# Septimus4/semi-supervised-image-processing

Hardware: AMD Instinct MI355X
Metric: images/sec semi-supervised train step, 224x224 bs=256, 1/2/4/8 MI355X (higher is better)
Workload: dtype bf16; 1 GPU; semi_consistency_resnet18_224; model=resnet18, global_batch=256, per_gpu_batch=256, labeled_per_gpu=128, unlabeled_per_gpu=128, image_size=224, parallelism=dp1

## Files before the change

semi-supervised-image-processing_amd/csrc/optim.hip:

```cpp
#include "ssip_common.h"

namespace {

struct AdamC {
  float decay, w1, b2, eps, step_size, bc2_sqrt, grad_scale;
};

__device__ __forceinline__ void adamw_math(float& pi, float& mi, float& vi, float graw, const AdamC& c) {
#pragma clang fp contract(off)
  const float gi = graw * c.grad_scale;
  pi = pi * c.decay;
  mi = (c.w1 < 0.5f) ? mi + c.w1 * (gi - mi) : gi - (gi - mi) * (1.f - c.w1);
  vi = vi * c.b2 + (1.f - c.b2) * gi * gi;
  const float denom = sqrtf(vi) / c.bc2_sqrt + c.eps;
  pi = pi - c.step_size * (mi / denom);
}

__device__ __forceinline__ void adamw_scalar(long i, float* __restrict__ p, const float* __restrict__ g,
                                             float* __restrict__ m, float* __restrict__ v, const AdamC& c) {
  float pi = p[i], mi = m[i], vi = v[i];
  adamw_math(pi, mi, vi, g[i], c);
  p[i] = pi;
  m[i] = mi;
  v[i] = vi;
}

__device__ __forceinline__ void adamw_range(long n, float* __restrict__ p, const float* __restrict__ g,
                                            float* __restrict__ m, float* __restrict__ v, const AdamC& c) {
  const long tid = blockIdx.x * (long)blockDim.x + threadIdx.x, nt = (long)gridDim.x * blockDim.x;
  const uintptr_t a = reinterpret_cast<uintptr_t>(p) & 15;
  const bool vec = (reinterpret_cast<uintptr_t>(g) & 15) == a && (reinterpret_cast<uintptr_t>(m) & 15) == a &&
                   (reinterpret_cast<uintptr_t>(v) & 15) == a && (a & 3) == 0;
  const long head = vec ? min(n, (long)(((16 - a) & 15) >> 2)) : n;
  for (long i = tid; i < head; i += nt) adamw_scalar(i, p, g, m, v, c);
  if (!vec) return;
  const long nv = (n - head) >> 2;
  float4* __restrict__ p4 = reinterpret_cast<float4*>(p + head);
  const float4* __restrict__ g4 = reinterpret_cast<const float4*>(g + head);
  float4* __restrict__ m4 = reinterpret_cast<float4*>(m + head);
  float4* __restrict__ v4 = reinterpret_cast<float4*>(v + head);
  for (long j = tid; j < nv; j += 2 * nt) {
    const long j1 = j + nt < nv ? j + nt : j;
    float4 pp[2] = {p4[j], p4[j1]}, mm[2] = {m4[j], m4[j1]}, vv[2] = {v4[j], v4[j1]};
    const float4 gg[2] = {g4[j], g4[j1]};
    asm volatile("" ::: "memory");
#pragma unroll
    for (int u = 0; u < 2; ++u) {
      adamw_math(pp[u].x, mm[u].x, vv[u].x, gg[u].x, c);
      adamw_math(pp[u].y, mm[u].y, vv[u].y, gg[u].y, c);
      adamw_math(pp[u].z, mm[u].z, vv[u].z, gg[u].z, c);
      adamw_math(pp[u].w, mm[u].w, vv[u].w, gg[u].w, c);
    }
    p4[j] = pp[0];
    m4[j] = mm[0];
    v4[j] = vv[0];
    if (j1 != j) {
      p4[j1] = pp[1];
      m4[j1] = mm[1];
      v4[j1] = vv[1];
    }
  }
  for (long i = head + (nv << 2) + tid; i < n; i += nt) adamw_scalar(i, p, g, m, v, c);
}

__global__ void adamw_kernel(long n, float* __restrict__ p, const float* __restrict__ g, float* __restrict__ m,
                             float* __restrict__ v, float lr, float b1, float b2, float eps, float wd, float step_size,
                             float bc2_sqrt, float grad_scale) {
  const AdamC c{1.f - lr * wd, 1.f - b1, b2, eps, step_size, bc2_sqrt, grad_scale};
  adamw_range(n, p, g, m, v, c);
}

__global__ void adamw_sched_kernel(double* sched, double b1, double b2) {
  const double t = sched[1] + 1.0;
  sched[1] = t;
  sched[2] = sched[0] / (1.0 - pow(b1, t));
  sched[3] = sqrt(1.0 - pow(b2, t));
  sched[5] = 1.0 - pow(b1, t + 1.0);
  sched[6] = sqrt(1.0 - pow(b2, t + 1.0));
}

__global__ void adamw_dev_kernel(long n, float* __restrict__ p, const float* __restrict__ g, float* __restrict__ m,
                                 float* __restrict__ v, double* sched, float b1, float b2, float eps, float wd,
                                 float grad_scale, int advance) {
  double t = sched[1], ss = sched[2], bc = sched[3];
  if (advance) {
    t += 1.0;
    const double c1 = sched[5];
    if (c1 != 0.0) {
      ss = sched[0] / c1;
      bc = sched[6];
    } else {
      ss = sched[0] / (1.0 - pow((double)b1, t));
      bc = sqrt(1.0 - pow((double)b2, t));
    }
  }
  const float lr = (float)sched[0];
  const AdamC c{1.f - lr * wd, 1.f - b1, b2, eps, (float)ss, (float)bc, grad_scale};
  adamw_range(n, p, g, m, v, c);
  if (advance) {
    __syncthreads();
    if (threadIdx.x != 0) return;
    unsigned long long* cnt = reinterpret_cast<unsigned long long*>(sched + 4);
    const unsigned long long old = __hip_atomic_fetch_add(cnt, 1ull, __ATOMIC_RELAXED, __HIP_MEMORY_SCOPE_AGENT);
    if (old == gridDim.x - 1) {
      sched[1] = t;
      sched[2] = ss;
      sched[3] = bc;
      sched[5] = 1.0 - pow((double)b1, t + 1.0);
      sched[6] = sqrt(1.0 - pow((double)b2, t + 1.0));
      __hip_atomic_store(cnt, 0ull, __ATOMIC_RELAXED, __HIP_MEMORY_SCOPE_AGENT);
    }
  }
}

template <typename T>
__global__ void weight_prep_kernel(int K, int C, int R, int S, int Cp, int Sp, const float* __restrict__ w,
                                   T* __restrict__ krsc, T* __restrict__ crsk) {
  const long total = (long)K * R * Sp * Cp;
  for (long i = blockIdx.x * (long)blockDim.x + threadIdx.x; i < total; i += (long)gridDim.x * blockDim.x) {
    const int c = (int)(i % Cp);
    long t = i / Cp;
    const int s = (int)(t % Sp);
    t /= Sp;
    const int r = (int)(t % R);
    const int k = (int)(t / R);
    const float v = (c < C && s < S) ? w[(((long)k * C + c) * R + r) * S + s] : 0.f;
    const T tv = from_f32<T>(v);
    if (krsc) krsc[i] = tv;
    if (crsk) crsk[(((long)c * R + r) * Sp + s) * K + k] = tv;
  }
}

struct WprepTable {
  ssip_wprep it[SSIP_WPREP_MAX];
  int tile_start[SSIP_WPREP_MAX + 1];
  int count;
  int xcd;
};

template <typename T>
__global__ void __launch_bounds__(256) weight_prep_batch_kernel(const WprepTable tab) {
  __shared__ float tile[64][65];
  int b = blockIdx.x, idx = 0;
  if (tab.xcd) {
    const int nb = gridDim.x, xcd = b & 7, q = nb >> 3, r = nb & 7;
    b = xcd * q + min(xcd, r) + (b >> 3);
  }
  while (idx + 1 < tab.count && b >= tab.tile_start[idx + 1]) ++idx;
  const ssip_wprep& e = tab.it[idx];
  b -= tab.tile_start[idx];
  const int rs = b % (e.R * e.Sp);
  b /= e.R * e.Sp;
  const int r = rs / e.Sp, s = rs - r * e.Sp;
  const int ctiles = (e.Cp + 63) / 64;
  const int k0 = (b / ctiles) * 64, c0 = (b % ctiles) * 64;
  const int tx = threadIdx.x & 63, ty = threadIdx.x >> 6;
  T* krsc = static_cast<T*>(e.w_krsc);
  T* crsk = static_cast<T*>(e.w_crsk);
  float vals[16];
#pragma unroll
  for (int q = 0; q < 16; ++q) {
    const int k = k0 + ty + 4 * q, c = c0 + tx;
    vals[q] = (k < e.K && c < e.C && s < e.S) ? e.w_kcrs[(((long)k * e.C + c) * e.R + r) * e.S + s] : 0.f;
  }
#pragma unroll
  for (int q = 0; q < 16; ++q) {
    const int k = k0 + ty + 4 * q;
    float v = vals[q];
    if (e.kscale && k < e.K && c0 + tx < e.C && s < e.S) v *= e.kscale[k];
    tile[ty + 4 * q][tx] = v;
  }
  __syncthreads();
  if (krsc) {
    for (int kk = ty; kk < 64; kk += 4) {
      const int k = k0 + kk, c = c0 + tx;
      if (k < e.K && c < e.Cp) krsc[(((long)k * e.R + r) * e.Sp + s) * e.Cp + c] = from_f32<T>(tile[kk][tx]);
    }
  }
  if (crsk) {
    for (int cc = ty; cc < 64; cc += 4) {
      const int c = c0 + cc, k = k0 + tx;
      if (k < e.K && c < e.Cp) crsk[(((long)c * e.R + r) * e.Sp + s) * e.K + k] = from_f32<T>(tile[tx][cc]);
    }
  }
}

}

extern "C" {

int ssip_adamw(int64_t n, float* param, const float* grad, float* exp_avg, float* exp_avg_sq, float lr, float beta1,
               float beta2, float eps, float weight_decay, int64_t step, float grad_scale, void* stream) {
  SSIP_REQUIRE(n > 0 && param && grad && exp_avg && exp_avg_sq && step >= 1, SSIP_ERR_ARG, "ssip_adamw: bad arguments");
  const double bc1 = 1.0 - pow((double)beta1, (double)step);
  const double bc2 = 1.0 - pow((double)beta2, (double)step);
  const float step_size = (float)((double)lr / bc1);
  const float bc2_sqrt = (float)sqrt(bc2);
  long blocks = (n + 1023) / 1024;
  if (blocks > 8192) blocks = 8192;
  SSIP_KLAUNCH(adamw_kernel, dim3((int)blocks), dim3(256), 0, (hipStream_t)stream, (long)n, param, grad, exp_avg,
                     exp_avg_sq, lr, beta1, beta2, eps, weight_decay, step_size, bc2_sqrt, grad_scale);
  return ::ssip::check_launch("adamw");
}

int ssip_adamw_sched_step(double* sched, float beta1, float beta2, void* stream) {
  SSIP_REQUIRE(sched, SSIP_ERR_ARG, "ssip_adamw_sched_step: null schedule");
  SSIP_KLAUNCH(adamw_sched_kernel, dim3(1), dim3(1), 0, (hipStream_t)stream, sched, (double)beta1,
                     (double)beta2);
  return ::ssip::check_launch("adamw_sched");
}

int ssip_adamw_dev(int64_t n, float* param, const float* grad, float* exp_avg, float* exp_avg_sq, double* sched,
                   float beta1, float beta2, float eps, float weight_decay, float grad_scale, int advance,
                   void* stream) {
  SSIP_REQUIRE(n > 0 && param && grad && exp_avg && exp_avg_sq && sched, SSIP_ERR_ARG,
               "ssip_adamw_dev: bad arguments");
  long blocks = (n + 1023) / 1024;
  if (blocks > 2048) blocks = 2048;
  SSIP_KLAUNCH(adamw_dev_kernel, dim3((int)blocks), dim3(256), 0, (hipStream_t)stream, (long)n, param, grad,
                     exp_avg, exp_avg_sq, sched, beta1, beta2, eps, weight_decay, grad_scale, advance ? 1 : 0);
  return ::ssip::check_launch("adamw_dev");
}

int ssip_weight_prep(int dtype, int K, int C, int R, int S, int Cp, int Sp, const float* w_kcrs, void* w_krsc,
                     void* w_crsk, void* stream) {
  SSIP_REQUIRE(K > 0 && C > 0 && R > 0 && S > 0 && Cp >= C && Sp >= S && w_kcrs && (w_krsc || w_crsk), SSIP_ERR_ARG,
               "ssip_weight_prep: bad arguments");
  const long total = (long)K * R * Sp * Cp;
  long blocks = (total + 255) / 256;
  if (blocks > 8192) blocks = 8192;
  SSIP_DISPATCH_DTYPE(dtype, T, {
    SSIP_KLAUNCH(weight_prep_kernel<T>, dim3((int)blocks), dim3(256), 0, (hipStream_t)stream, K, C, R, S, Cp, Sp,
                       w_kcrs, (T*)w_krsc, (T*)w_crsk);
  });
  return ::ssip::check_launch("weight_prep");
}

}

extern "C" int ssip_weight_prep_batch(int dtype, int count, const ssip_wprep* items, void* stream) {
  SSIP_REQUIRE(count >= 0 && count <= SSIP_WPREP_MAX && (count == 0 || items), SSIP_ERR_ARG,
               "ssip_weight_prep_batch: count must be 0..%d", SSIP_WPREP_MAX);
  if (count == 0) return SSIP_OK;
  WprepTable tab;
  memset(&tab, 0, sizeof(tab));
  tab.count = count;
  int tiles = 0;
  for (int i = 0; i < count; ++i) {
    const ssip_wprep& e = items[i];
    SSIP_REQUIRE(e.K > 0 && e.C > 0 && e.R > 0 && e.S > 0 && e.Cp >= e.C && e.Sp >= e.S && e.w_kcrs &&
                     (e.w_krsc || e.w_crsk),
                 SSIP_ERR_ARG, "ssip_weight_prep_batch: bad item %d", i);
    tab.it[i] = e;
    tab.tile_start[i] = tiles;
    tiles += ((e.K + 63) / 64) * ((e.Cp + 63) / 64) * e.R * e.Sp;
  }
  tab.tile_start[count] = tiles;
  tab.xcd = 1;
  SSIP_DISPATCH_DTYPE(dtype, T, {
    SSIP_KLAUNCH(weight_prep_batch_kernel<T>, dim3(tiles), dim3(256), 0, (hipStream_t)stream, tab);
  });
  return ::ssip::check_launch("weight_prep_batch");
}

namespace {
struct CounterTable {
  int64_t* p[SSIP_COUNTERS_MAX];
};

__global__ void counters_add_kernel(CounterTable t, int count, int64_t delta) {
  const int i = threadIdx.x;
  if (i < count) t.p[i][0] += delta;
}
}

extern "C" int ssip_counters_add(int count, int64_t* const* ptrs, int64_t delta, void* stream) {
  SSIP_REQUIRE(count >= 0 && count <= SSIP_COUNTERS_MAX && (count == 0 || ptrs), SSIP_ERR_ARG,
               "ssip_counters_add: count must be 0..%d", SSIP_COUNTERS_MAX);
  if (count == 0) return SSIP_OK;
  CounterTable t;
  for (int i = 0; i < count; ++i) {
    SSIP_REQUIRE(ptrs[i], SSIP_ERR_ARG, "ssip_counters_add: null counter %d", i);
    t.p[i] = ptrs[i];
  }
  SSIP_KLAUNCH(counters_add_kernel, dim3(1), dim3(64), 0, (hipStream_t)stream, t, count, delta);
  return ::ssip::check_launch("counters_add");
}
```

Before: 44180 images/s.

## Retile batched weight prep to read contiguous KCRS rows with float4 and vectorized stores

The batched weight-layout kernel now tiles over K and C only, with every R,S position inside one tile. Each block loads whole contiguous KCRS rows with aligned float4 reads into a padded LDS tile. It then writes the KRSC and CRSK layouts with 16-byte packed stores where alignment allows. This replaces strided scalar gathers (one tile per r,s position) with coalesced vector traffic and fewer, larger blocks, at the cost of more complex index walking and LDS-size-driven tile selection on the host.

```diff
diff --git a/semi-supervised-image-processing_amd/csrc/optim.hip b/semi-supervised-image-processing_amd/csrc/optim.hip
--- a/semi-supervised-image-processing_amd/csrc/optim.hip
+++ b/semi-supervised-image-processing_amd/csrc/optim.hip
@@ -131,57 +131,167 @@
   }
 }
 
+constexpr int kWprepLdsElems = 9472;
+constexpr int kWprepMaxVec = 10;
+
 struct WprepTable {
   ssip_wprep it[SSIP_WPREP_MAX];
   int tile_start[SSIP_WPREP_MAX + 1];
+  unsigned char tk[SSIP_WPREP_MAX], tc[SSIP_WPREP_MAX];
   int count;
-  int xcd;
 };
+
+__host__ __device__ inline int wprep_kstride(int c, int rs, int esize) {
+  int ks = c * rs;
+  while (esize == 2 ? (ks & 3) != 2 : !(ks & 1)) ++ks;
+  return ks;
+}
+
+__host__ __device__ inline bool wprep_tile_fits(int tk, int tc, int C, int rs, int esize) {
+  const int c = tc < C ? tc : C;
+  return tk * wprep_kstride(c, rs, esize) <= kWprepLdsElems && tk * ((c * rs + 6) / 4) <= 256 * kWprepMaxVec;
+}
+
+template <typename T, int W>
+struct alignas(sizeof(T) * W) WprepPack {
+  T e[W];
+};
+
+struct WprepWalk {
+  int hi, r, s, lo, dhi, dr, ds, dlo, R, Sp, n;
+  __device__ __forceinline__ WprepWalk(int v, int R_, int Sp_, int n_) : R(R_), Sp(Sp_), n(n_) {
+    split(v, hi, r, s, lo);
+    split(256, dhi, dr, ds, dlo);
+  }
+  __device__ __forceinline__ void split(int v, int& h, int& r_, int& s_, int& l) const {
+    l = v % n;
+    v /= n;
+    s_ = v % Sp;
+    v /= Sp;
+    r_ = v % R;
+    h = v / R;
+  }
+  __device__ __forceinline__ void next() {
+    lo += dlo;
+    if (lo >= n) lo -= n, ++s;
+    s += ds;
+    if (s >= Sp) s -= Sp, ++r;
+    r += dr;
+    if (r >= R) r -= R, ++hi;
+    hi += dhi;
+  }
+};
+
+template <typename T, int W>
+__device__ __forceinline__ void wprep_store_krsc(const ssip_wprep& e, const T* tile, int ks, int k0, int c0, int tke,
+                                                 int nc, int wc) {
+  T* krsc = static_cast<T*>(e.w_krsc);
+  const int RS = e.R * e.S, cv = wc / W, nv = tke * e.R * e.Sp * cv;
+  WprepWalk w(threadIdx.x, e.R, e.Sp, cv);
+  for (int v = threadIdx.x; v < nv; v += 256, w.next()) {
+    const int cl = w.lo * W;
+    const T* src = tile + w.hi * ks + w.r * e.S + w.s;
+    WprepPack<T, W> p;
+#pragma unroll
+    for (int j = 0; j < W; ++j) p.e[j] = (w.s < e.S && cl + j < nc) ? src[(cl + j) * RS] : from_f32<T>(0.f);
+    *reinterpret_cast<WprepPack<T, W>*>(krsc + (((k0 + w.hi) * e.R + w.r) * e.Sp + w.s) * e.Cp + c0 + cl) = p;
+  }
+}
+
+template <typename T, int W>
+__device__ __forceinline__ void wprep_store_crsk(const ssip_wprep& e, const T* tile, int ks, int k0, int c0, int tke,
+                                                 int nc, int wc) {
+  T* crsk = static_cast<T*>(e.w_crsk);
+  const int RS = e.R * e.S, kv = tke / W, nv = wc * e.R * e.Sp * kv;
+  WprepWalk w(threadIdx.x, e.R, e.Sp, kv);
+  for (int v = threadIdx.x; v < nv; v += 256, w.next()) {
+    const int kk = w.lo * W;
+    const T* src = tile + kk * ks + w.hi * RS + w.r * e.S + w.s;
+    const bool in = w.s < e.S && w.hi < nc;
+    WprepPack<T, W> p;
+#pragma unroll
+    for (int j = 0; j < W; ++j) p.e[j] = in ? src[j * ks] : from_f32<T>(0.f);
+    *reinterpret_cast<WprepPack<T, W>*>(crsk + (((c0 + w.hi) * e.R + w.r) * e.Sp + w.s) * e.K + k0 + kk) = p;
+  }
+}
 
 template <typename T>
 __global__ void __launch_bounds__(256) weight_prep_batch_kernel(const WprepTable tab) {
-  __shared__ float tile[64][65];
+  __shared__ T tile[kWprepLdsElems];
+  constexpr int VE = 16 / (int)sizeof(T);
   int b = blockIdx.x, idx = 0;
-  if (tab.xcd) {
+  {
     const int nb = gridDim.x, xcd = b & 7, q = nb >> 3, r = nb & 7;
     b = xcd * q + min(xcd, r) + (b >> 3);
   }
   while (idx + 1 < tab.count && b >= tab.tile_start[idx + 1]) ++idx;
   const ssip_wprep& e = tab.it[idx];
   b -= tab.tile_start[idx];
-  const int rs = b % (e.R * e.Sp);
-  b /= e.R * e.Sp;
-  const int r = rs / e.Sp, s = rs - r * e.Sp;
-  const int ctiles = (e.Cp + 63) / 64;
-  const int k0 = (b / ctiles) * 64, c0 = (b % ctiles) * 64;
-  const int tx = threadIdx.x & 63, ty = threadIdx.x >> 6;
-  T* krsc = static_cast<T*>(e.w_krsc);
-  T* crsk = static_cast<T*>(e.w_crsk);
-  float vals[16];
-#pragma unroll
-  for (int q = 0; q < 16; ++q) {
-    const int k = k0 + ty + 4 * q, c = c0 + tx;
-    vals[q] = (k < e.K && c < e.C && s < e.S) ? e.w_kcrs[(((long)k * e.C + c) * e.R + r) * e.S + s] : 0.f;
-  }
-#pragma unroll
-  for (int q = 0; q < 16; ++q) {
-    const int k = k0 + ty + 4 * q;
-    float v = vals[q];
-    if (e.kscale && k < e.K && c0 + tx < e.C && s < e.S) v *= e.kscale[k];
-    tile[ty + 4 * q][tx] = v;
+  const int TK = tab.tk[idx], TC = tab.tc[idx];
+  const int ktiles = (e.K + TK - 1) / TK;
+  const int k0 = (b % ktiles) * TK, c0 = (b / ktiles) * TC;
+  const int RS = e.R * e.S;
+  const int tke = min(TK, e.K - k0);
+  const int nc = max(0, min(TC, e.C - c0));
+  const int wc = min(TC, e.Cp - c0);
+  const int rl = nc * RS;
+  const int ks = wprep_kstride(min(TC, e.C), RS, (int)sizeof(T));
+  const int spr = (rl + 6) >> 2, nslots = tke * spr;
+  const int total = e.K * e.C * RS;
+  const int mis = (int)((reinterpret_cast<uintptr_t>(e.w_kcrs) >> 2) & 3);
+  float4 vals[kWprepMaxVec];
+  float sc[kWprepMaxVec];
+  const int kk0 = threadIdx.x / spr, j0 = threadIdx.x - kk0 * spr, dk = 256 / spr, dj = 256 - dk * spr;
+  int kk = kk0, j = j0;
+#pragma unroll
+  for (int q = 0; q < kWprepMaxVec; ++q) {
+    vals[q] = make_float4(0.f, 0.f, 0.f, 0.f);
+    sc[q] = 1.f;
+    const int lo = ((k0 + kk) * e.C + c0) * RS;
+    const int e0 = lo - ((lo + mis) & 3) + 4 * j;
+    if (threadIdx.x + 256 * q < nslots && e0 < lo + rl) {
+      if (e.kscale) sc[q] = e.kscale[k0 + kk];
+      if (e0 >= 0 && e0 + 4 <= total) {
+        vals[q] = *reinterpret_cast<const float4*>(e.w_kcrs + e0);
+      } else {
+        if (e0 >= 0 && e0 < total) vals[q].x = e.w_kcrs[e0];
+        if (e0 + 1 >= 0 && e0 + 1 < total) vals[q].y = e.w_kcrs[e0 + 1];
+        if (e0 + 2 >= 0 && e0 + 2 < total) vals[q].z = e.w_kcrs[e0 + 2];
+        if (e0 + 3 >= 0 && e0 + 3 < total) vals[q].w = e.w_kcrs[e0 + 3];
+      }
+    }
+    j += dj;
+    if (j >= spr) j -= spr, ++kk;
+    kk += dk;
+  }
+  kk = kk0, j = j0;
+#pragma unroll
+  for (int q = 0; q < kWprepMaxVec; ++q) {
+    if (threadIdx.x + 256 * q < nslots) {
+      const int lo = ((k0 + kk) * e.C + c0) * RS;
+      const int off = 4 * j - ((lo + mis) & 3);
+      const float v4[4] = {vals[q].x, vals[q].y, vals[q].z, vals[q].w};
+#pragma unroll
+      for (int i = 0; i < 4; ++i) {
+        if (off + i >= 0 && off + i < rl) tile[kk * ks + off + i] = from_f32<T>(e.kscale ? v4[i] * sc[q] : v4[i]);
+      }
+    }
+    j += dj;
+    if (j >= spr) j -= spr, ++kk;
+    kk += dk;
   }
   __syncthreads();
-  if (krsc) {
-    for (int kk = ty; kk < 64; kk += 4) {
-      const int k = k0 + kk, c = c0 + tx;
-      if (k < e.K && c < e.Cp) krsc[(((long)k * e.R + r) * e.Sp + s) * e.Cp + c] = from_f32<T>(tile[kk][tx]);
-    }
-  }
-  if (crsk) {
-    for (int cc = ty; cc < 64; cc += 4) {
-      const int c = c0 + cc, k = k0 + tx;
-      if (k < e.K && c < e.Cp) crsk[(((long)c * e.R + r) * e.Sp + s) * e.K + k] = from_f32<T>(tile[tx][cc]);
-    }
+  if (e.w_krsc) {
+    if (wc % VE == 0 && e.Cp % VE == 0 && (reinterpret_cast<uintptr_t>(e.w_krsc) & 15) == 0)
+      wprep_store_krsc<T, VE>(e, tile, ks, k0, c0, tke, nc, wc);
+    else
+      wprep_store_krsc<T, 1>(e, tile, ks, k0, c0, tke, nc, wc);
+  }
+  if (e.w_crsk) {
+    if (TK % VE == 0 && e.K % VE == 0 && (reinterpret_cast<uintptr_t>(e.w_crsk) & 15) == 0)
+      wprep_store_crsk<T, VE>(e, tile, ks, k0, c0, tke, nc, wc);
+    else
+      wprep_store_crsk<T, 1>(e, tile, ks, k0, c0, tke, nc, wc);
   }
 }
 
@@ -242,23 +352,33 @@
   SSIP_REQUIRE(count >= 0 && count <= SSIP_WPREP_MAX && (count == 0 || items), SSIP_ERR_ARG,
                "ssip_weight_prep_batch: count must be 0..%d", SSIP_WPREP_MAX);
   if (count == 0) return SSIP_OK;
+  const int esize = dtype == SSIP_F32 ? 4 : 2;
   WprepTable tab;
   memset(&tab, 0, sizeof(tab));
   tab.count = count;
-  int tiles = 0;
+  long tiles = 0;
   for (int i = 0; i < count; ++i) {
     const ssip_wprep& e = items[i];
     SSIP_REQUIRE(e.K > 0 && e.C > 0 && e.R > 0 && e.S > 0 && e.Cp >= e.C && e.Sp >= e.S && e.w_kcrs &&
                      (e.w_krsc || e.w_crsk),
                  SSIP_ERR_ARG, "ssip_weight_prep_batch: bad item %d", i);
+    const long rs = (long)e.R * e.S;
+    SSIP_REQUIRE(rs <= kWprepLdsElems - 4, SSIP_ERR_ARG, "ssip_weight_prep_batch: item %d: filter too large", i);
+    SSIP_REQUIRE((long)e.K * e.C * rs < (1l << 31) && (long)e.K * e.R * e.Sp * e.Cp < (1l << 31), SSIP_ERR_ARG,
+                 "ssip_weight_prep_batch: item %d: more than 2^31 elements", i);
+    int tk = rs == 1 ? 64 : 16, tc = 64;
+    while (tk > 1 && !wprep_tile_fits(tk, tc, e.C, (int)rs, esize)) tk >>= 1;
+    while (tc > 1 && !wprep_tile_fits(tk, tc, e.C, (int)rs, esize)) tc >>= 1;
     tab.it[i] = e;
-    tab.tile_start[i] = tiles;
-    tiles += ((e.K + 63) / 64) * ((e.Cp + 63) / 64) * e.R * e.Sp;
-  }
-  tab.tile_start[count] = tiles;
-  tab.xcd = 1;
+    tab.tk[i] = (unsigned char)tk;
+    tab.tc[i] = (unsigned char)tc;
+    tab.tile_start[i] = (int)tiles;
+    tiles += (long)((e.K + tk - 1) / tk) * ((e.Cp + tc - 1) / tc);
+    SSIP_REQUIRE(tiles < (1l << 30), SSIP_ERR_ARG, "ssip_weight_prep_batch: item %d: too many tiles", i);
+  }
+  tab.tile_start[count] = (int)tiles;
   SSIP_DISPATCH_DTYPE(dtype, T, {
-    SSIP_KLAUNCH(weight_prep_batch_kernel<T>, dim3(tiles), dim3(256), 0, (hipStream_t)stream, tab);
+    SSIP_KLAUNCH(weight_prep_batch_kernel<T>, dim3((int)tiles), dim3(256), 0, (hipStream_t)stream, tab);
   });
   return ::ssip::check_launch("weight_prep_batch");
 }
```

Measured after the change: 44220 images/s, median of 3. No clear change (+0.1%).
